# google-research/multinerf

Measured on NVIDIA H100. Metric: train-step rays/sec @16384 rays x (64+64+32) samples, higher is better.
Workload: dtype bf16

## Files before the change

### include/mnrf.h

```cpp
#ifndef MNRF_H_
#define MNRF_H_

#include <stddef.h>
#include <stdint.h>

#ifdef __cplusplus
extern "C" {
#endif

typedef uint16_t mnrf_bf16;
typedef void* mnrf_stream;

#define MNRF_ABI_VERSION 2

int mnrf_abi_version(void);
const char* mnrf_last_error(void);
int mnrf_device_ok(void);
int mnrf_num_sms(void);

typedef struct {
  int32_t num_rays, num_prev, num_samples;
  int32_t use_dilation;
  float dilation, domain_lo, domain_hi;
  float anneal, resample_padding;
// ... 54 lines not shown
                    const float* side_w, float* side_aw, float* out, mnrf_stream stream);

typedef struct {
  int32_t block_n;
  int32_t staged;
  int32_t mask_tma;
  int32_t smooth;
  int32_t side;
  int32_t splits;
  int32_t tiles;
  int32_t grid;
  int32_t pingpong;
  int32_t epilogue;
} mnrf_gemm_instance;
int mnrf_gemm_plan(const mnrf_gemm_desc* d, const mnrf_bf16* a, const mnrf_bf16* b, const float* bias,
                   const float* rowv, const float* colv, const mnrf_bf16* mask, const uint32_t* maskbits,
                   const float* colsum, const mnrf_bf16* addend, const mnrf_bf16* z, int64_t ldz, const void* out,
                   const float* bsum, const float* side_w, const float* side_aw, mnrf_gemm_instance* plan);

#define MNRF_CHAIN_MAX_LAYERS 8
enum { MNRF_CHAIN_FWD = 0, MNRF_CHAIN_BWD = 1 };

typedef struct {
  const mnrf_bf16* w;
  int64_t ldw;
  const float* bias;
  uint32_t* maskbits;
  int64_t ldmaskbits;
  float* colsum;
  mnrf_bf16* out;
  int64_t ldo;
  int32_t n_stream, stream_col0, stream_kb0;
  int32_t n_res, res_kb0;
  int32_t reserved;
} mnrf_chain_layer;

typedef struct {
  int32_t mode, num_layers;
  int32_t width;
  int32_t stream_cols;
  int64_t m;
  const mnrf_bf16* stream;
  int64_t ldstream;
  const float* head_w;
  const float* head_b;
  float* head_out;
  int32_t head_n;
  int32_t reserved;
  mnrf_chain_layer layer[MNRF_CHAIN_MAX_LAYERS];
} mnrf_chain_desc;

int mnrf_mlp_chain(const mnrf_chain_desc* d, mnrf_stream stream);
int mnrf_mlp_chain_max_layers(void);

int mnrf_head_fwd(int64_t m, int32_t k, int32_t n_out, const mnrf_bf16* x, int64_t ldx,
                  const mnrf_bf16* w, const float* b, float* raw, mnrf_stream stream);
int mnrf_head_bwd(int64_t m, int32_t k, int32_t n_out, const mnrf_bf16* x, int64_t ldx,
                  const mnrf_bf16* w, const float* draw, mnrf_bf16* dx, int64_t lddx,
                  int32_t act, const mnrf_bf16* z, int64_t ldz, float* dw, float* dw2, int32_t dw_split,
                  float* db, float* dxsum, int32_t dx_cols, mnrf_bf16* dx2, int64_t lddx2, mnrf_stream stream);

enum { MNRF_HEAD_NONE = 0, MNRF_HEAD_FWD_SUB = 1, MNRF_HEAD_FWD_WARP = 2, MNRF_HEAD_BWD_SUB = 3,
       MNRF_HEAD_BWD_WARP = 4 };
typedef struct {
  int32_t fwd_kernel;
  int32_t fwd_lpr;
  int32_t fwd_grid;
  int32_t bwd_kernel;
  int32_t bwd_n_out;
  int32_t bwd_lpr;
  int32_t bwd_chunks;
  int32_t bwd_smooth;
  int32_t bwd_grid;
  int32_t reserved;
  int64_t fwd_rows_per_pass;
  int64_t bwd_rows_per_block;
} mnrf_head_instance;
int mnrf_head_plan(int64_t m, int32_t k, int32_t n_out, const mnrf_bf16* x, const mnrf_bf16* w, int32_t act,
                   const mnrf_bf16* z, const mnrf_bf16* dx, mnrf_head_instance* plan);

int mnrf_colsum(int64_t m, int32_t n, const mnrf_bf16* x, int64_t ldx, float* out,
                mnrf_stream stream);

enum { MNRF_RGB_SIGMOID = 0, MNRF_RGB_SAFE_EXP = 1 };

typedef struct {
  int32_t num_rays, num_samples;
  int32_t raydist_fn, opaque_background;
  float density_bias, density_noise;
  int32_t rgb_act;
  float rgb_premult, rgb_bias, rgb_padding;
  float bg_const;
  int32_t rgb_mode;
  int32_t ld_density, ld_rgb;
} mnrf_composite_desc;

int mnrf_composite_fwd(const mnrf_composite_desc* d, const float* raw_density,
                       const float* raw_rgb, const float* density_noise, const float* sdist,
                       const float* directions, const float* near, const float* far,
                       const float* bg_rgb, const float* rgb_scale, const float* raw_diffuse,
                       const float* raw_tint, float* weights, float* rgb_out,
                       float* density_out, float* rgb_samples, float* acc, float* dist,
                       mnrf_stream stream);

int mnrf_point_rgb(const mnrf_composite_desc* d, int64_t M, const float* raw_rgb, int32_t ld_rgb,
                   const float* raw_diffuse, const float* raw_tint, float* rgb_out, mnrf_stream stream);
// ... 198 lines not shown
```

### multinerf_b200/csrc/chain.cu

```cuda
#include <stdlib.h>
#include <string.h>

#include <algorithm>

#include "tc_common.cuh"

namespace mnrf {

constexpr int CH_W = 256;
constexpr int CH_ROWS = 128;
constexpr int CH_KBLK = CH_ROWS * 128;
constexpr int CH_WBLK = CH_W * 128;
constexpr int CH_RING = 4;
constexpr int CH_SEG = CH_W / 64;
constexpr int CH_SBLK = 64 * 128;
constexpr int CH_SRING = 3;
constexpr int CH_ACT = 4 * CH_KBLK;
constexpr int CH_THREADS = 384;
constexpr int CH_MAX_LAYERS = MNRF_CHAIN_MAX_LAYERS;
constexpr int CH_AUX = CH_MAX_LAYERS * CH_W * 4;
constexpr int CH_SMEM = CH_ACT + CH_RING * CH_WBLK + CH_SRING * CH_SBLK + CH_AUX + 256  + 1024 ;
static_assert(CH_SMEM <= 232448, "shared memory budget");
static_assert(CH_SEG >= 1 && CH_SEG <= CH_RING, "a segment must fit in the weight ring");

struct alignas(64) ChainMaps {
  CUtensorMap stream;
  CUtensorMap w[CH_MAX_LAYERS];
  CUtensorMap out[CH_MAX_LAYERS];
};

struct ChainLayer {
  int n_stream, stream_col0, stream_kb0;
  int n_res, res_kb0;
  int store;
  const float* bias;
  uint32_t* maskbits;
  int64_t ldmaskbits;
  float* colsum;
};

struct ChainParams {
  int num_layers;
  int64_t m;
  int64_t num_units;
  ChainLayer layer[CH_MAX_LAYERS];
  const float* head_w;
  const float* head_b;
  float* head_out;
};

__device__ __forceinline__ uint32_t pack_bf16_relu(float lo, float hi) {
  uint32_t r;
  asm("cvt.rn.relu.bf16x2.f32 %0, %1, %2;" : "=r"(r) : "f"(hi), "f"(lo));
  return r;
}

__device__ __forceinline__ float2 ld_shared_const_f2(uint32_t addr) {
  float2 v;
  asm("ld.shared.v2.f32 {%0, %1}, [%2];" : "=f"(v.x), "=f"(v.y) : "r"(addr));
  return v;
}

enum { CK_TURN, CK_FULL, CK_MMA, CK_EPI_SYNC, CK_EPI_LOOP, CK_EPI_TAIL, CK_N };
#ifdef MNRF_CHAIN_CLOCKS
__device__ unsigned long long g_chain_clk[CK_N];
#define CH_CLK(k) do { const long long t_ = clock64(); clk[k] += t_ - clk_t; clk_t = t_; } while (0)
#else
#define CH_CLK(k) do { } while (0)
#endif

template <int MODE, int NH>
__global__ void __launch_bounds__(CH_THREADS, 1)
mlp_chain_kernel(const __grid_constant__ ChainMaps maps, const ChainParams p) {
  extern __shared__ uint8_t smem_dyn[];
  uint8_t* smem = reinterpret_cast<uint8_t*>((reinterpret_cast<uintptr_t>(smem_dyn) + 1023) & ~uintptr_t(1023));
  uint8_t* act = smem;
  uint8_t* wring = act + CH_ACT;
  uint8_t* sring = wring + CH_RING * CH_WBLK;
  float* aux = reinterpret_cast<float*>(sring + CH_SRING * CH_SBLK);
  uint64_t* wfull = reinterpret_cast<uint64_t*>(aux + CH_MAX_LAYERS * CH_W);
  uint64_t* wempty = wfull + CH_RING;
  uint64_t* sfull = wempty + CH_RING;
  uint64_t* sempty = sfull + CH_SRING;
  uint64_t* turn = sempty + CH_SRING;

  const int warp = threadIdx.x >> 5;
  const int lane = threadIdx.x & 31;
  const int wg = threadIdx.x >> 7;

  if (threadIdx.x == 0) {
    bool any_stream = false;
    for (int j = 0; j < p.num_layers; ++j) {
      prefetch_tmap(&maps.w[j]);
      if (p.layer[j].store) prefetch_tmap(&maps.out[j]);
      any_stream |= p.layer[j].n_stream > 0;
    }
    if (any_stream) prefetch_tmap(&maps.stream);
    for (int i = 0; i < CH_RING; ++i) { mbar_init(&wfull[i], 1); mbar_init(&wempty[i], 8); }
    for (int i = 0; i < CH_SRING; ++i) { mbar_init(&sfull[i], 1); mbar_init(&sempty[i], 4); }
    for (int i = 0; i < 2; ++i) mbar_init(&turn[i], 4);
    fence_barrier_init();
  }
  if (MODE == 1)
    for (int i = threadIdx.x; i < CH_MAX_LAYERS * CH_W; i += CH_THREADS) aux[i] = 0.f;
  __syncthreads();
  pdl_launch_dependents();
  pdl_wait();
  if (MODE == 0) {
    for (int i = threadIdx.x; i < p.num_layers * CH_W; i += CH_THREADS) aux[i] = __ldg(p.layer[i / CH_W].bias + i % CH_W);
    __syncthreads();
  }

  if (wg == 0) {
    setmaxnreg_dec<40>();
    if (threadIdx.x == 0) {
      uint32_t wslot = 0, wphase = 0, sslot = 0, sphase = 0;
      for (int64_t unit = blockIdx.x; unit < p.num_units; unit += gridDim.x) {
        const int row0 = (int)(unit * CH_ROWS);
        for (int j = 0; j < p.num_layers; ++j) {
          const ChainLayer& L = p.layer[j];
          const int nk = L.n_res + L.n_stream;
          for (int s0 = 0; s0 < nk; s0 += CH_SEG) {
            const int s1 = min(s0 + CH_SEG, nk);
            for (int c = 0; c < 2; ++c)
              for (int s = s0; s < s1; ++s) {
                const bool streamed = s >= L.n_res;
                const int si = s - L.n_res;
                if (c == 0) {
                  mbar_wait(&wempty[wslot], wphase ^ 1, 1);
                  mbar_expect_tx(&wfull[wslot], CH_WBLK);
                  tma_load_2d(wring + wslot * CH_WBLK, &maps.w[j], &wfull[wslot],
                              (streamed ? L.stream_kb0 + si : L.res_kb0 + s) * 64, 0);
                  if (++wslot == CH_RING) { wslot = 0; wphase ^= 1; }
                }
                if (streamed) {
                  mbar_wait(&sempty[sslot], sphase ^ 1, 2);
                  mbar_expect_tx(&sfull[sslot], CH_SBLK);
                  tma_load_2d(sring + sslot * CH_SBLK, &maps.stream, &sfull[sslot], L.stream_col0 + si * 64, row0 + 64 * c);
                  if (++sslot == CH_SRING) { sslot = 0; sphase ^= 1; }
                }
              }
          }
          if (j == 0 && L.n_stream > 0 && unit + gridDim.x < p.num_units)
            for (int si = 0; si < L.n_stream; ++si)
              for (int c = 0; c < 2; ++c)
                tma_prefetch_2d(&maps.stream, L.stream_col0 + si * 64, (int)((unit + gridDim.x) * CH_ROWS) + 64 * c);
        }
      }
    }
  } else {
    setmaxnreg_inc<232>();
    const int c = wg - 1;
    const int w = warp & 3;
    const int r_in = 64 * c + 16 * w + (lane >> 2);
    const int q = lane & 3;
    const int cq = 2 * q;
    const uint32_t wring_s = smem_u32(wring), sring_s = smem_u32(sring), act_s = smem_u32(act);
    const uint32_t aux_s = smem_u32(aux);
    const bool lead = (threadIdx.x & 127) == 0;
    uint32_t wslot = 0, wphase = 0;
    uint32_t spos = 0;
    uint32_t seg = 0;
#ifdef MNRF_CHAIN_CLOCKS
    long long clk[CK_N] = {};
    long long clk_t = clock64();
#endif
    float acc[CH_W / 2];
    for (int64_t unit = blockIdx.x; unit < p.num_units; unit += gridDim.x) {
      int64_t rows[2];
      bool row_ok[2];
#pragma unroll
      for (int h = 0; h < 2; ++h) {
        rows[h] = unit * CH_ROWS + r_in + 8 * h;
        row_ok[h] = rows[h] < p.m;
      }
      for (int j = 0; j < p.num_layers; ++j) {
        const ChainLayer& L = p.layer[j];
        const bool last = (j == p.num_layers - 1);
        const bool do_head = (MODE == 0) && last && p.head_w != nullptr;
        uint32_t mw[2][2] = {{0u, 0u}, {0u, 0u}};
        if (MODE == 1 && L.maskbits) {
#pragma unroll
          for (int h = 0; h < 2; ++h)
#pragma unroll
            for (int e = 0; e < 2; ++e)
              if (row_ok[h]) mw[h][e] = __ldg(L.maskbits + rows[h] * L.ldmaskbits + 2 * q + e);
        }
        const int nk = L.n_res + L.n_stream;
        fence_acc(acc);
        for (int s0 = 0; s0 < nk; s0 += CH_SEG, ++seg) {
          const int s1 = min(s0 + CH_SEG, nk);
          const int ns = s1 - max(s0, L.n_res);
          uint32_t sp = spos + (c && ns > 0 ? ns : 0);
          if (ns > 0) spos += 2 * ns;
          if (c == 1) mbar_wait(&turn[1], seg & 1, 7);
          else if (seg > 0) mbar_wait(&turn[0], (seg - 1) & 1, 7);
          CH_CLK(CK_TURN);
          int prev_w = -1, prev_s = -1;
          for (int s = s0; s < s1; ++s) {
            const bool streamed = s >= L.n_res;
            mbar_wait(&wfull[wslot], wphase, 3);
            uint32_t a0 = act_s + s * CH_KBLK + c * (64 * 128);
            int cur_s = -1;
            if (streamed) {
              cur_s = (int)(sp % CH_SRING);
              mbar_wait(&sfull[cur_s], (sp / CH_SRING) & 1, 4);
              a0 = sring_s + cur_s * CH_SBLK;
              ++sp;
            }
            CH_CLK(CK_FULL);
            const uint32_t b0 = wring_s + wslot * CH_WBLK;
            wgmma_fence();
#pragma unroll
            for (int k = 0; k < 64 / WGMMA_K; ++k)
              Wgmma<CH_W, 0, 0>::mma(acc, make_smem_desc(a0 + k * (WGMMA_K * 2), 0, 1024),
                                     make_smem_desc(b0 + k * (WGMMA_K * 2), 0, 1024), (s > 0 || k > 0) ? 1u : 0u);
            wgmma_commit();
            wgmma_wait<1>();
            if (lane == 0) {
              if (prev_w >= 0) mbar_arrive(&wempty[prev_w]);
              if (prev_s >= 0) mbar_arrive(&sempty[prev_s]);
            }
            prev_w = (int)wslot;
            prev_s = cur_s;
            if (++wslot == CH_RING) { wslot = 0; wphase ^= 1; }
          }
          __syncwarp();
          if (lane == 0) mbar_arrive(&turn[c ^ 1]);
          wgmma_wait<0>();
          if (lane == 0) {
            mbar_arrive(&wempty[prev_w]);
            if (prev_s >= 0) mbar_arrive(&sempty[prev_s]);
          }
          CH_CLK(CK_MMA);
        }
        fence_acc(acc);

        if (lead) tma_store_wait_read<0>();
        named_bar_sync(1 + c, 128);
        CH_CLK(CK_EPI_SYNC);
        uint32_t bits[2] = {0u, 0u};
        float hdot[NH][2];
#pragma unroll
        for (int o = 0; o < NH; ++o) hdot[o][0] = hdot[o][1] = 0.f;
#pragma unroll
        for (int i = 0; i < CH_W / 8; ++i) {
          const int col = 8 * i + cq;
          float v[2][2];
#pragma unroll
          for (int h = 0; h < 2; ++h) { v[h][0] = acc[4 * i + 2 * h]; v[h][1] = acc[4 * i + 2 * h + 1]; }
          uint32_t o[2];
          if (MODE == 0) {
            const float2 b = ld_shared_const_f2(aux_s + (j * CH_W + col) * 4);
#pragma unroll
            for (int h = 0; h < 2; ++h) {
              v[h][0] += b.x;
              v[h][1] += b.y;
              bits[h] |= ((v[h][0] > 0.f ? 1u : 0u) | (v[h][1] > 0.f ? 2u : 0u)) << (col & 31);
              o[h] = pack_bf16_relu(v[h][0], v[h][1]);
            }
            if (do_head) {
#pragma unroll
              for (int oo = 0; oo < NH; ++oo) {
                const float2 hw = __ldg(reinterpret_cast<const float2*>(p.head_w + oo * CH_W + col));
#pragma unroll
                for (int h = 0; h < 2; ++h) hdot[oo][h] += bf16_lo(o[h]) * hw.x + bf16_hi(o[h]) * hw.y;
              }
            }
          } else {
            if (L.maskbits && (i & 3) == 0) {
#pragma unroll
              for (int h = 0; h < 2; ++h)
                bits[h] = __shfl_sync(0xffffffffu, mw[h][(i >> 2) & 1], (lane & ~3) | (i >> 3));
            }
#pragma unroll
            for (int h = 0; h < 2; ++h) {
              if (L.maskbits) {
                if (!((bits[h] >> (col & 31)) & 1u)) v[h][0] = 0.f;
                if (!((bits[h] >> ((col + 1) & 31)) & 1u)) v[h][1] = 0.f;
              }
              o[h] = pack_bf16(v[h][0], v[h][1]);
            }
            if (L.colsum) {
              float s0 = v[0][0] + v[1][0], s1 = v[0][1] + v[1][1];
#pragma unroll
              for (int sh = 4; sh < 32; sh <<= 1) {
                s0 += __shfl_xor_sync(0xffffffffu, s0, sh);
                s1 += __shfl_xor_sync(0xffffffffu, s1, sh);
              }
              if (lane < 4) { atomicAdd(aux + j * CH_W + col, s0); atomicAdd(aux + j * CH_W + col + 1, s1); }
            }
          }
#pragma unroll
          for (int h = 0; h < 2; ++h) {
            const int r = r_in + 8 * h;
            st_shared_u32(act_s + (col >> 6) * CH_KBLK + r * 128 + ((((col & 63) >> 3) ^ (r & 7)) << 4) + (cq << 1), o[h]);
          }
          if (MODE == 0 && (i & 3) == 3) {
#pragma unroll
            for (int h = 0; h < 2; ++h) {
              bits[h] |= __shfl_xor_sync(0xffffffffu, bits[h], 1);
              bits[h] |= __shfl_xor_sync(0xffffffffu, bits[h], 2);
              if (q == (i >> 3)) mw[h][(i >> 2) & 1] = bits[h];
              bits[h] = 0u;
            }
          }
        }
        CH_CLK(CK_EPI_LOOP);
        fence_proxy_async();
        named_bar_sync(1 + c, 128);
        CH_CLK(CK_EPI_SYNC);
        if (lead && L.store) {
#pragma unroll
          for (int kb = 0; kb < 4; ++kb)
            tma_store_2d(&maps.out[j], act + kb * CH_KBLK + c * (64 * 128), kb * 64, (int)(unit * CH_ROWS) + 64 * c);
          tma_store_commit();
        }
        if (MODE == 0 && L.maskbits) {
          const bool wide = (((uintptr_t)L.maskbits | (uintptr_t)(L.ldmaskbits * 4)) & 7) == 0;
#pragma unroll
          for (int h = 0; h < 2; ++h) {
            if (!row_ok[h]) continue;
            uint32_t* dst = L.maskbits + rows[h] * L.ldmaskbits + 2 * q;
            if (wide) *reinterpret_cast<uint2*>(dst) = make_uint2(mw[h][0], mw[h][1]);
            else { dst[0] = mw[h][0]; dst[1] = mw[h][1]; }
          }
        }
        if (do_head) {
#pragma unroll
          for (int oo = 0; oo < NH; ++oo)
#pragma unroll
            for (int h = 0; h < 2; ++h) {
              hdot[oo][h] += __shfl_xor_sync(0xffffffffu, hdot[oo][h], 1);
              hdot[oo][h] += __shfl_xor_sync(0xffffffffu, hdot[oo][h], 2);
              if (q == 0 && row_ok[h])
                p.head_out[rows[h] * NH + oo] = hdot[oo][h] + (p.head_b ? __ldg(p.head_b + oo) : 0.f);
            }
        }
        CH_CLK(CK_EPI_TAIL);
      }
    }
    if (lead) tma_store_wait_all();
#ifdef MNRF_CHAIN_CLOCKS
    if (blockIdx.x == 0 && threadIdx.x == 256)
      for (int k = 0; k < CK_N; ++k) atomicAdd(&g_chain_clk[k], (unsigned long long)clk[k]);
#endif
    if (MODE == 1) {
      named_bar_sync(3, 256);
      for (int jj = 0; jj < p.num_layers; ++jj) {
        if (!p.layer[jj].colsum) continue;
        for (int i = threadIdx.x - 128; i < CH_W; i += 256) atomicAdd(p.layer[jj].colsum + i, aux[jj * CH_W + i]);
      }
    }
  }
}

}

extern "C" int mnrf_mlp_chain_max_layers(void) { return mnrf::CH_MAX_LAYERS; }

#ifdef MNRF_CHAIN_CLOCKS
extern "C" int mnrf_chain_clocks(unsigned long long* out) {
  unsigned long long zero[mnrf::CK_N] = {};
  if (cudaDeviceSynchronize() != cudaSuccess) return 1;
  if (cudaMemcpyFromSymbol(out, mnrf::g_chain_clk, sizeof(zero)) != cudaSuccess) return 1;
  return cudaMemcpyToSymbol(mnrf::g_chain_clk, zero, sizeof(zero)) != cudaSuccess;
}
#endif

extern "C" int mnrf_mlp_chain(const mnrf_chain_desc* d, mnrf_stream stream_) {
  using namespace mnrf;
  cudaStream_t stream = (cudaStream_t)stream_;
  MNRF_CHECK(d, "mnrf_mlp_chain: null descriptor");
  MNRF_CHECK(d->m >= 0 && (d->m + CH_ROWS - 1) / CH_ROWS * CH_ROWS <= INT32_MAX,
             "mnrf_mlp_chain: m must be in [0, %d], got %lld", INT32_MAX / CH_ROWS * CH_ROWS, (long long)d->m);
  if (d->m == 0) return 0;
  MNRF_CHECK(d->mode == MNRF_CHAIN_FWD || d->mode == MNRF_CHAIN_BWD, "mnrf_mlp_chain: bad mode %d", d->mode);
  MNRF_CHECK(d->num_layers >= 1 && d->num_layers <= CH_MAX_LAYERS, "mnrf_mlp_chain: 1..%d layers, got %d",
             CH_MAX_LAYERS, d->num_layers);
  MNRF_CHECK(d->width == CH_W, "mnrf_mlp_chain: layer width must be %d, got %d", CH_W, d->width);
  const int sms = mnrf_num_sms();
  ChainMaps maps;
  memset(&maps, 0, sizeof(maps));
  ChainParams p{};
  p.num_layers = d->num_layers;
  p.m = d->m;
  p.num_units = (d->m + CH_ROWS - 1) / CH_ROWS;
  bool any_stream = false;
  for (int j = 0; j < d->num_layers; ++j) {
    const mnrf_chain_layer& s = d->layer[j];
    ChainLayer& L = p.layer[j];
    MNRF_CHECK(s.n_res == 0 || s.n_res == CH_W / 64, "mnrf_mlp_chain: layer %d: n_res must be 0 or %d", j, CH_W / 64);
    MNRF_CHECK(s.n_stream >= 0 && (s.n_stream > 0 || s.n_res > 0), "mnrf_mlp_chain: layer %d has no operand", j);
    MNRF_CHECK(s.stream_col0 >= 0 && s.stream_kb0 >= 0 && s.res_kb0 >= 0,
               "mnrf_mlp_chain: layer %d: negative column or k-block offset", j);
    MNRF_CHECK(j > 0 || s.n_res == 0, "mnrf_mlp_chain: the first layer has no resident operand");
    MNRF_CHECK(s.w && ((uintptr_t)s.w % 16) == 0 && s.ldw % 8 == 0, "mnrf_mlp_chain: layer %d: weights must be 16-byte aligned", j);
    const int kblocks = std::max(s.n_stream > 0 ? s.stream_kb0 + s.n_stream : 0, s.n_res > 0 ? s.res_kb0 + s.n_res : 0);
    MNRF_CHECK(s.ldw >= (int64_t)kblocks * 64, "mnrf_mlp_chain: layer %d: weight pitch %lld < K %d", j, (long long)s.ldw, kblocks * 64);
    L.n_stream = s.n_stream; L.stream_col0 = s.stream_col0; L.stream_kb0 = s.stream_kb0;
    L.n_res = s.n_res; L.res_kb0 = s.res_kb0;
    L.store = s.out ? 1 : 0;
    L.bias = s.bias; L.maskbits = s.maskbits; L.ldmaskbits = s.ldmaskbits; L.colsum = s.colsum;
    if (s.bias) MNRF_CHECK(((uintptr_t)s.bias % 8) == 0, "mnrf_mlp_chain: layer %d: bias must be 8-byte aligned", j);
    if (s.maskbits)
      MNRF_CHECK(s.ldmaskbits >= CH_W / 32, "mnrf_mlp_chain: layer %d: maskbits rows must hold >= %d words", j, CH_W / 32);
    if (d->mode == MNRF_CHAIN_BWD) MNRF_CHECK(!s.bias, "mnrf_mlp_chain: bias is a forward input");
    else MNRF_CHECK(s.bias && !s.colsum, "mnrf_mlp_chain: layer %d: the forward chain takes a bias and no colsum", j);
    if (make_tmap(&maps.w[j], s.w, CH_W, (int64_t)kblocks * 64, s.ldw, 64, CH_W)) return 1;
    if (s.out) {
      MNRF_CHECK(((uintptr_t)s.out % 16) == 0 && s.ldo % 8 == 0 && s.ldo >= CH_W, "mnrf_mlp_chain: layer %d: output alignment", j);
      if (make_tmap(&maps.out[j], s.out, d->m, CH_W, s.ldo, 64, 64)) return 1;
    }
    any_stream |= s.n_stream > 0;
    if (s.n_stream > 0)
      MNRF_CHECK(s.stream_col0 % 64 == 0 && s.stream_col0 + s.n_stream * 64 <= d->stream_cols,
                 "mnrf_mlp_chain: layer %d: streamed columns [%d, %d) outside the stream tensor (%d columns)", j,
                 s.stream_col0, s.stream_col0 + s.n_stream * 64, d->stream_cols);
  }
  if (any_stream) {
    MNRF_CHECK(d->stream && ((uintptr_t)d->stream % 16) == 0 && d->ldstream % 8 == 0 && d->stream_cols % 64 == 0,
               "mnrf_mlp_chain: streamed operand must be 16-byte aligned with a multiple of 64 columns");
    MNRF_CHECK(d->ldstream >= d->stream_cols, "mnrf_mlp_chain: stream pitch %lld < %d columns",
               (long long)d->ldstream, d->stream_cols);
    if (make_tmap(&maps.stream, d->stream, d->m, d->stream_cols, d->ldstream, 64, CH_ROWS / 2)) return 1;
  }
  p.head_w = d->head_w; p.head_b = d->head_b; p.head_out = d->head_out;
  const int head_n = d->head_n ? d->head_n : 1;
  if (d->head_w) MNRF_CHECK(d->mode == MNRF_CHAIN_FWD && d->head_out && ((uintptr_t)d->head_w % 16) == 0,
                            "mnrf_mlp_chain: the head is a forward output (16-byte aligned weights)");
  MNRF_CHECK(head_n == 1 || (head_n == 4 && d->head_w), "mnrf_mlp_chain: head_n must be 1 or 4, got %d", head_n);
  const int grid = (int)std::min<int64_t>(p.num_units, sms);
  const int rc = d->mode == MNRF_CHAIN_BWD ? launch_tc<mlp_chain_kernel<1, 1>>(grid, CH_THREADS, CH_SMEM, stream, maps, p)
                 : head_n == 4             ? launch_tc<mlp_chain_kernel<0, 4>>(grid, CH_THREADS, CH_SMEM, stream, maps, p)
                                           : launch_tc<mlp_chain_kernel<0, 1>>(grid, CH_THREADS, CH_SMEM, stream, maps, p);
  if (rc) return rc;
  MNRF_LAUNCH_CHECK();
  return 0;
}
```

### multinerf_b200/lib.py

```python
import ctypes as C
import os

import torch

_HERE = os.path.dirname(os.path.abspath(__file__))
LIB_PATH = os.environ.get('MNRF_LIB') or os.path.join(_HERE, 'libmnrf_b200.so')


class MnrfError(RuntimeError):
  pass


class SampleDesc(C.Structure):
  _fields_ = [('num_rays', C.c_int32), ('num_prev', C.c_int32), ('num_samples', C.c_int32),
              ('use_dilation', C.c_int32), ('dilation', C.c_float), ('domain_lo', C.c_float),
              ('domain_hi', C.c_float), ('anneal', C.c_float), ('resample_padding', C.c_float),
              ('jitter_mode', C.c_int32), ('max_jitter', C.c_float)]


class EncodeDesc(C.Structure):
  _fields_ = [('num_rays', C.c_int32), ('num_samples', C.c_int32), ('raydist_fn', C.c_int32),
              ('ray_shape', C.c_int32), ('warp_contract', C.c_int32),
              ('disable_integration', C.c_int32), ('basis_k', C.c_int32), ('min_deg', C.c_int32),
              ('max_deg', C.c_int32), ('ld_feat', C.c_int32), ('feat_cols', C.c_int32)]
# ... 32 lines not shown
  _fields_ = [('c', CompositeDesc), ('loss_type', C.c_int32), ('charb_padding', C.c_float),
              ('data_mult', C.c_float), ('distortion_mult', C.c_float),
              ('interlevel_mult', C.c_float), ('num_samples_fine', C.c_int32),
              ('lossmult_channels', C.c_int32)]


class RobustDesc(C.Structure):
  _fields_ = [('num_rays', C.c_int32), ('patch_size', C.c_int32), ('inner_patch_size', C.c_int32),
              ('filter_size', C.c_int32), ('enable', C.c_int32), ('smoothed_thresh', C.c_float),
              ('patch_thresh', C.c_float)]


class RefdirDesc(C.Structure):
  _fields_ = [('M', C.c_int64), ('num_samples', C.c_int32), ('use_pred_normals', C.c_int32),
              ('use_density_normals', C.c_int32), ('use_reflections', C.c_int32), ('use_ide', C.c_int32),
              ('use_n_dot_v', C.c_int32), ('use_roughness', C.c_int32), ('deg_view', C.c_int32),
              ('ide_n', C.c_int32), ('roughness_bias', C.c_float), ('ld', C.c_int32), ('col0', C.c_int32),
              ('col_end', C.c_int32)]


class CameraDesc(C.Structure):
  _fields_ = [('num_rays', C.c_int32), ('num_cameras', C.c_int32), ('camtype', C.c_int32),
              ('has_distortion', C.c_int32), ('k1', C.c_float), ('k2', C.c_float), ('k3', C.c_float),
              ('k4', C.c_float), ('p1', C.c_float), ('p2', C.c_float), ('undistort_eps', C.c_float),
              ('undistort_iters', C.c_int32), ('has_ndc', C.c_int32), ('ndc_p02', C.c_float),
              ('ndc_p12', C.c_float), ('ndc_near', C.c_float)]


class SphericalDesc(C.Structure):
  _fields_ = [('height', C.c_int32), ('width', C.c_int32), ('camtoworld', C.c_double * 12)]


class PackItem(C.Structure):
  _fields_ = [('master', C.c_void_p), ('w_nk', C.c_void_p), ('w_kn', C.c_void_p), ('in_pad', C.c_int32),
              ('out', C.c_int32), ('tile0', C.c_int32), ('reserved', C.c_int32)]


CHAIN_MAX_LAYERS = 8
CHAIN_FWD, CHAIN_BWD = 0, 1


class ChainLayer(C.Structure):
  _fields_ = [('w', C.c_void_p), ('ldw', C.c_int64), ('bias', C.c_void_p), ('maskbits', C.c_void_p),
              ('ldmaskbits', C.c_int64), ('colsum', C.c_void_p), ('out', C.c_void_p), ('ldo', C.c_int64),
              ('n_stream', C.c_int32), ('stream_col0', C.c_int32), ('stream_kb0', C.c_int32),
              ('n_res', C.c_int32), ('res_kb0', C.c_int32), ('reserved', C.c_int32)]


class ChainDesc(C.Structure):
  _fields_ = [('mode', C.c_int32), ('num_layers', C.c_int32), ('width', C.c_int32), ('stream_cols', C.c_int32),
              ('m', C.c_int64), ('stream', C.c_void_p), ('ldstream', C.c_int64), ('head_w', C.c_void_p),
              ('head_b', C.c_void_p), ('head_out', C.c_void_p), ('head_n', C.c_int32), ('reserved', C.c_int32),
              ('layer', ChainLayer * CHAIN_MAX_LAYERS)]


class AdamDesc(C.Structure):
  _fields_ = [('n', C.c_int64), ('grad_max_val', C.c_float), ('grad_max_norm', C.c_float),
              ('lr', C.c_float), ('beta1', C.c_float), ('beta2', C.c_float), ('eps', C.c_float),
              ('step', C.c_int32), ('grad_scale', C.c_float)]


RAYDIST = {None: 0, 'none': 0, 'reciprocal': 1, 'log': 2, 'exp': 3, 'sqrt': 4, 'square': 5,
           'piecewise': 6}
RAY_SHAPE = {'cone': 0, 'cylinder': 1}
RGB_ACT = {'sigmoid': 0, 'safe_exp': 1}
LOSS_TYPE = {'mse': 0, 'charb': 1, 'rawnerf': 2}
GEMM_FWD, GEMM_DGRAD, GEMM_WGRAD = 0, 1, 2
ACT_NONE, ACT_RELU, ACT_SOFTPLUS, ACT_SILU = 0, 1, 2, 3
SMOOTH_ACTS = (ACT_SOFTPLUS, ACT_SILU)

_P = C.c_void_p
_SIGNATURES = {
    'mnrf_abi_version': (C.c_int, []),
    'mnrf_last_error': (C.c_char_p, []),
    'mnrf_device_ok': (C.c_int, []),
    'mnrf_num_sms': (C.c_int, []),
    'mnrf_sample_level': (C.c_int, [C.POINTER(SampleDesc)] + [_P] * 12),
    'mnrf_encode': (C.c_int, [C.POINTER(EncodeDesc)] + [_P] * 11 + [C.c_int32, _P]),
    'mnrf_viewdir_enc': (C.c_int, [C.c_int32, C.c_int32, C.c_int32, _P, _P, C.c_int32, C.c_int32,
                                   C.c_int32, _P]),
    'mnrf_gemm': (C.c_int, [C.POINTER(GemmDesc)] + [_P] * 10 + [C.c_int64, _P, _P]),
    'mnrf_gemm_wgrad': (C.c_int, [C.POINTER(GemmDesc)] + [_P] * 7),
    'mnrf_gemm_plan': (C.c_int, [C.POINTER(GemmDesc)] + [_P] * 10 + [C.c_int64] + [_P] * 4 +
                       [C.POINTER(GemmInstance)]),
    'mnrf_mlp_chain': (C.c_int, [C.POINTER(ChainDesc), _P]),
    'mnrf_mlp_chain_max_layers': (C.c_int, []),
    'mnrf_head_fwd': (C.c_int, [C.c_int64, C.c_int32, C.c_int32, _P, C.c_int64, _P, _P, _P, _P]),
    'mnrf_head_bwd': (C.c_int, [C.c_int64, C.c_int32, C.c_int32, _P, C.c_int64, _P, _P, _P, C.c_int64, C.c_int32,
                                _P, C.c_int64, _P, _P, C.c_int32, _P, _P, C.c_int32, _P, C.c_int64, _P]),
    'mnrf_head_plan': (C.c_int, [C.c_int64, C.c_int32, C.c_int32, _P, _P, C.c_int32, _P, _P, _P]),
    'mnrf_colsum': (C.c_int, [C.c_int64, C.c_int32, _P, C.c_int64, _P, _P]),
    'mnrf_composite_fwd': (C.c_int, [C.POINTER(CompositeDesc)] + [_P] * 18),
    'mnrf_composite_bwd': (C.c_int, [C.POINTER(LossDesc)] + [_P] * 24 + [C.c_int32, _P]),
    'mnrf_robust_mask': (C.c_int, [C.POINTER(RobustDesc)] + [_P] * 7 + [C.c_int32, _P]),
    'mnrf_quantile': (C.c_int, [C.c_int32, C.c_float, _P, _P, _P]),
    'mnrf_refdir_fwd': (C.c_int, [C.POINTER(RefdirDesc)] + [_P] * 10 + [C.c_float, C.c_float, C.c_int32, _P, _P]),
    'mnrf_refdir_bwd': (C.c_int, [C.POINTER(RefdirDesc)] + [_P] * 8 + [C.c_int32, C.c_float, C.c_float, C.c_int32] +
                        [_P] * 8),
    'mnrf_normals_fwd': (C.c_int, [C.c_int64, C.c_int32] + [_P] * 5 + [C.c_float, C.c_float, C.c_int32, _P, _P]),
    'mnrf_normals_bwd': (C.c_int, [C.c_int64, C.c_int32] + [_P] * 4 + [C.c_float, C.c_float, C.c_int32] + [_P] * 2 +
                         [C.c_int64] + [_P] * 3 +
                         [C.c_int64, _P, _P]),
    'mnrf_outer_mask': (C.c_int,[C.c_int64, C.c_int32, C.c_int64, _P, _P, _P, C.c_int64, _P, C.c_int64, _P]),
    'mnrf_act_tangent_bwd': (C.c_int, [C.c_int64, C.c_int32, C.c_int32] + [_P, C.c_int64] * 5 + [C.c_int32, _P]),
    'mnrf_pixels_to_rays': (C.c_int, [C.POINTER(CameraDesc)] + [_P] * 11),
    'mnrf_spherical_rays': (C.c_int, [C.POINTER(SphericalDesc)] + [_P] * 6),
    'mnrf_clip_adam': (C.c_int, [C.POINTER(AdamDesc)] + [_P] * 7),
    'mnrf_pack_weights_batched': (C.c_int, [C.c_int32, _P, C.c_int32, _P]),
    'mnrf_encode_points': (C.c_int, [C.POINTER(EncodeDesc), _P, C.c_float, _P, _P, _P, _P]),
    'mnrf_marching_cubes': (C.c_int, [C.c_int32] * 4 + [_P, C.c_float] + [_P] * 7),
    'mnrf_encode_points_tangent': (C.c_int, [C.POINTER(EncodeDesc), _P, C.c_float, _P, _P, _P, C.c_int32, _P]),
    'mnrf_point_rgb': (C.c_int, [C.POINTER(CompositeDesc), C.c_int64, _P, C.c_int32, _P, _P, _P, _P]),
    'mnrf_mc_normals': (C.c_int, [C.c_int32] * 3 + [_P, C.c_float] + [_P] * 4),
    'mnrf_tsdf_integrate': (C.c_int, [C.POINTER(CameraDesc)] + [C.c_int32] * 3 + [C.c_double] * 4 + [C.c_int32] * 3 +
                            [_P] * 5 + [C.c_float] + [_P] * 5),
    'mnrf_tsdf_integrate_contracted': (C.c_int, [C.POINTER(CameraDesc)] + [C.c_int32] * 3 + [C.c_double] * 4 +
                                       [C.c_int32] * 3 + [_P] * 5 + [C.c_float] + [_P] * 5),
    'mnrf_mesh_uncontract': (C.c_int, [C.c_int64] + [_P] * 5),
    'mnrf_mesh_components': (C.c_int, [C.c_int32, C.c_int64, _P, _P, _P]),
    'mnrf_points_view_count': (C.c_int, [C.POINTER(CameraDesc), C.c_int64, _P, C.c_int32, C.c_int32, C.c_int32,
                                         _P, _P, _P, _P]),
    'mnrf_mesh_quadrics': (C.c_int, [C.c_int32, C.c_int64] + [_P] * 4 + [C.c_int64] + [_P] * 6),
    'mnrf_mesh_edge_cost': (C.c_int, [C.c_int32, C.c_int64, C.c_int64] + [_P] * 12),
    'mnrf_mesh_collapse_select': (C.c_int, [C.c_int32, C.c_int64, C.c_int64] + [_P] * 7),
    'mnrf_mesh_collapse_apply': (C.c_int, [C.c_int32, C.c_int64, C.c_int64] + [_P] * 13),
    'mnrf_mesh_texture_raster': (C.c_int, [C.c_int32, C.c_int64, _P, _P, _P, C.c_int32] + [_P] * 5),
    'mnrf_mesh_bvh': (C.c_int, [C.c_int32, C.c_int32, C.c_int64] + [_P] * 12),
    'mnrf_mesh_trace': (C.c_int, [C.c_int64] + [_P] * 4 + [C.c_int64] + [_P] * 9),
}
MC_COUNT, MC_EMIT = 0, 1
BVH_BOXES, BVH_KEYS, BVH_TREE = 0, 1, 2
HEAD_NONE, HEAD_FWD_SUB, HEAD_FWD_WARP, HEAD_BWD_SUB, HEAD_BWD_WARP = 0, 1, 2, 3, 4
EXPORTED = tuple(_SIGNATURES)

_lib = None


def load(build_if_missing=False):
  global _lib
# ... 45 lines not shown
```

### multinerf_b200/ops.py

```python
import ctypes as C
import math
from typing import NamedTuple

import torch

from . import lib as L

EPS = float(torch.finfo(torch.float32).eps)

LAUNCHES = 0
GEMM_EVENTS = None


def _count(n=1):
  global LAUNCHES
  LAUNCHES += n


def _gemm_call(flops, fn, *args):
  _count()
  if GEMM_EVENTS is None:
    L.check(fn(*args))
    return
  ev = (torch.cuda.Event(enable_timing=True), torch.cuda.Event(enable_timing=True))
# ... 433 lines not shown
  _gemm_call(2.0 * m * n * k, lib.mnrf_gemm_wgrad, C.byref(d), L.ptr(x), L.ptr(dy), L.ptr(bsum),
             L.ptr(_f32(side_w)), L.ptr(side_aw), L.ptr(out), L.stream_ptr())
  return out


def gemm_plan(mode, a, b, out, *, m, n, k, act=L.ACT_NONE, bias=None, rowv=None, colv=None, mask=None,
              maskbits=None, colsum=None, mask_mod=0, addend=None, z=None, bsum=None, side_w=None, side_aw=None):
  lib = L.load()
  def p(t):
    return None if t is None else C.c_void_p(t.data_ptr())
  def ld(t):
    return t.stride(0) if t is not None else 0
  d = L.GemmDesc(mode, act, m, n, k, a.stride(0), b.stride(0), out.stride(0), ld(mask), ld(maskbits), ld(addend),
                 mask_mod, 0)
  plan = L.GemmInstance()
  L.check(lib.mnrf_gemm_plan(C.byref(d), p(a), p(b), p(bias), p(rowv), p(colv), p(mask), p(maskbits), p(colsum),
                             p(addend), p(z), ld(z), p(out), p(bsum), p(side_w), p(side_aw), C.byref(plan)))
  return {name: int(getattr(plan, name)) for name, _ in L.GemmInstance._fields_}


def chain_desc(mode, m, layers, *, stream=None, stream_cols=0, head_w=None, head_b=None, head_out=None, head_n=1):
  d = L.ChainDesc()
  d.mode, d.num_layers, d.width, d.stream_cols, d.m = mode, len(layers), 256, stream_cols, m
  if stream is not None:
    assert stream.dtype == torch.bfloat16 and stream.stride(1) == 1
    d.stream, d.ldstream = stream.data_ptr(), stream.stride(0)
  if head_w is not None:
    assert head_w.is_contiguous() and head_w.numel() == head_n * 256 and head_out.is_contiguous()
    d.head_w, d.head_out, d.head_n = head_w.data_ptr(), head_out.data_ptr(), head_n
    d.head_b = head_b.data_ptr() if head_b is not None else None
  flops = 0.0
  for j, ly in enumerate(layers):
    c = d.layer[j]
    w = ly['w']
    assert w.dtype == torch.bfloat16 and w.stride(1) == 1
    c.w, c.ldw = w.data_ptr(), w.stride(0)
    for name in ('bias', 'colsum'):
      t = ly.get(name)
      setattr(c, name, t.data_ptr() if t is not None else None)
    mb = ly.get('maskbits')
    if mb is not None:
      assert mb.dtype == torch.int32 and mb.stride(1) == 1
      c.maskbits, c.ldmaskbits = mb.data_ptr(), mb.stride(0)
    out = ly.get('out')
    if out is not None:
      assert out.dtype == torch.bfloat16 and out.stride(1) == 1
      c.out, c.ldo = out.data_ptr(), out.stride(0)
    c.n_stream, c.stream_col0, c.stream_kb0 = ly.get('n_stream', 0), ly.get('stream_col0', 0), ly.get('stream_kb0', 0)
    c.n_res, c.res_kb0 = ly.get('n_res', 0), ly.get('res_kb0', 0)
    flops += 2.0 * m * 256 * 64 * (c.n_stream + c.n_res)
  return d, flops


def mlp_chain(desc):
  lib = L.load()
  d, flops = desc
  _gemm_call(flops, lib.mnrf_mlp_chain, C.byref(d), L.stream_ptr())


def head_fwd(x, w_nk, bias, n_out, k, raw=None):
  lib = L.load()
  M = x.shape[0]
  if raw is None:
    raw = torch.empty(M, n_out, device=x.device)
  _count()
  L.check(lib.mnrf_head_fwd(M, k, n_out, L.ptr(x), x.stride(0), L.ptr(w_nk), L.ptr(bias),
                            L.ptr(raw), L.stream_ptr()))
  return raw


def head_bwd(x, w_nk, draw, n_out, k, dx=None, relu_mask=False, dw=None, db=None, dxsum=None, dw2=None, dw_split=0,
             dx_cols=0, dx2=None, act=L.ACT_NONE, z=None):
  lib = L.load()
  M = x.shape[0]
  if z is not None:
    assert not relu_mask and z.dtype == torch.bfloat16 and z.stride(-1) == 1
  else:
    act = L.ACT_RELU if relu_mask else L.ACT_NONE
  _count()
  L.check(lib.mnrf_head_bwd(M, k, n_out, L.ptr(x), x.stride(0), L.ptr(w_nk), L.ptr(_f32(draw)),
                            L.ptr(dx), dx.stride(0) if dx is not None else 0, act,
                            L.ptr(z), z.stride(0) if z is not None else 0, L.ptr(dw), L.ptr(dw2), int(dw_split),
                            L.ptr(db), L.ptr(dxsum), int(dx_cols), L.ptr(dx2), dx2.stride(0) if dx2 is not None else 0,
                            L.stream_ptr()))


def head_plan(x, w_nk, n_out, k, *, act=L.ACT_NONE, z=None, dx=None):
  lib = L.load()
  def p(t):
    return None if t is None else C.c_void_p(t.data_ptr())
  plan = L.HeadInstance()
  L.check(lib.mnrf_head_plan(x.shape[0], k, n_out, p(x), p(w_nk), act, p(z), p(dx), C.byref(plan)))
  return {name: int(getattr(plan, name)) for name, _ in L.HeadInstance._fields_}


def colsum(x, n, out):
  lib = L.load()
  _count()
  L.check(lib.mnrf_colsum(x.shape[0], n, L.ptr(x), x.stride(0), L.ptr(out), L.stream_ptr()))


def _cdesc(B, S, *, raydist_fn, opaque_background, density_bias, density_noise, rgb_activation,
           rgb_premultiplier, rgb_bias, rgb_padding, bg_const, rgb_mode=0):
  if rgb_activation not in L.RGB_ACT:
    raise ValueError(f'rgb_activation {rgb_activation!r} not supported by the CUDA path')
  return L.CompositeDesc(B, S, L.RAYDIST[raydist_fn], int(opaque_background), float(density_bias),
# ... 214 lines not shown
```

Measured before the change: 293,300.

## Specialize backward chain epilogue for mask-only layers with TMA-loaded mask bits

Adds a template variant of the fused MLP chain kernel for backward passes where every layer has relu mask bits and no column sums. Mask words are prefetched per layer by the producer warp via TMA into a double-buffered shared area guarded by mbarriers, replacing per-thread global loads and shuffles. The column-sum zeroing and reduction are also compiled out. This adds barrier traffic and reuses the aux area, and falls back to an LDG variant when alignment does not allow TMA.

```diff
diff --git a/include/mnrf.h b/include/mnrf.h
--- a/include/mnrf.h
+++ b/include/mnrf.h
@@ -130,6 +130,12 @@
 
 int mnrf_mlp_chain(const mnrf_chain_desc* d, mnrf_stream stream);
 int mnrf_mlp_chain_max_layers(void);
+
+enum { MNRF_CHAIN_EPI_GENERIC = 0, MNRF_CHAIN_EPI_BITS = 1 };
+typedef struct {
+  int32_t epilogue, mask_tma, head_n, reserved;
+} mnrf_chain_instance;
+int mnrf_chain_plan(const mnrf_chain_desc* d, mnrf_chain_instance* plan);
 
 int mnrf_head_fwd(int64_t m, int32_t k, int32_t n_out, const mnrf_bf16* x, int64_t ldx,
                   const mnrf_bf16* w, const float* b, float* raw, mnrf_stream stream);
diff --git a/multinerf_b200/csrc/chain.cu b/multinerf_b200/csrc/chain.cu
--- a/multinerf_b200/csrc/chain.cu
+++ b/multinerf_b200/csrc/chain.cu
@@ -19,14 +19,22 @@
 constexpr int CH_THREADS = 384;
 constexpr int CH_MAX_LAYERS = MNRF_CHAIN_MAX_LAYERS;
 constexpr int CH_AUX = CH_MAX_LAYERS * CH_W * 4;
+constexpr int CH_MWORDS = CH_W / 32;
+constexpr int CH_MBLK = CH_ROWS * CH_MWORDS * 4;
+constexpr int CH_MBUFS = 2;
+static_assert(CH_MBUFS * CH_MBLK <= CH_AUX, "the mask blocks live in the column-sum area");
 constexpr int CH_SMEM = CH_ACT + CH_RING * CH_WBLK + CH_SRING * CH_SBLK + CH_AUX + 256  + 1024 ;
 static_assert(CH_SMEM <= 232448, "shared memory budget");
+static_assert((2 * CH_RING + 2 * CH_SRING + 2 + 2 * CH_MBUFS) * 8 <= 256, "barrier area");
+
+enum { CH_EPI_GENERIC = 0, CH_EPI_BITS_TMA = 1, CH_EPI_BITS_LDG = 2 };
 static_assert(CH_SEG >= 1 && CH_SEG <= CH_RING, "a segment must fit in the weight ring");
 
 struct alignas(64) ChainMaps {
   CUtensorMap stream;
   CUtensorMap w[CH_MAX_LAYERS];
   CUtensorMap out[CH_MAX_LAYERS];
+  CUtensorMap mask[CH_MAX_LAYERS];
 };
 
 struct ChainLayer {
@@ -69,9 +77,12 @@
 #define CH_CLK(k) do { } while (0)
 #endif
 
-template <int MODE, int NH>
+template <int MODE, int NH, int OPS>
 __global__ void __launch_bounds__(CH_THREADS, 1)
 mlp_chain_kernel(const __grid_constant__ ChainMaps maps, const ChainParams p) {
+  static_assert(OPS == CH_EPI_GENERIC || (MODE == 1 && NH == 1), "fixed operand sets are backward epilogues");
+  constexpr bool kFixed = OPS != CH_EPI_GENERIC;
+  constexpr bool kBitsTma = OPS == CH_EPI_BITS_TMA;
   extern __shared__ uint8_t smem_dyn[];
   uint8_t* smem = reinterpret_cast<uint8_t*>((reinterpret_cast<uintptr_t>(smem_dyn) + 1023) & ~uintptr_t(1023));
   uint8_t* act = smem;
@@ -83,6 +94,8 @@
   uint64_t* sfull = wempty + CH_RING;
   uint64_t* sempty = sfull + CH_SRING;
   uint64_t* turn = sempty + CH_SRING;
+  uint64_t* mfull = turn + 2;
+  uint64_t* mempty = mfull + CH_MBUFS;
 
   const int warp = threadIdx.x >> 5;
   const int lane = threadIdx.x & 31;
@@ -93,15 +106,18 @@
     for (int j = 0; j < p.num_layers; ++j) {
       prefetch_tmap(&maps.w[j]);
       if (p.layer[j].store) prefetch_tmap(&maps.out[j]);
+      if (kBitsTma) prefetch_tmap(&maps.mask[j]);
       any_stream |= p.layer[j].n_stream > 0;
     }
     if (any_stream) prefetch_tmap(&maps.stream);
     for (int i = 0; i < CH_RING; ++i) { mbar_init(&wfull[i], 1); mbar_init(&wempty[i], 8); }
     for (int i = 0; i < CH_SRING; ++i) { mbar_init(&sfull[i], 1); mbar_init(&sempty[i], 4); }
     for (int i = 0; i < 2; ++i) mbar_init(&turn[i], 4);
+    if (kBitsTma)
+      for (int i = 0; i < CH_MBUFS; ++i) { mbar_init(&mfull[i], 1); mbar_init(&mempty[i], 8); }
     fence_barrier_init();
   }
-  if (MODE == 1)
+  if (MODE == 1 && !kFixed)
     for (int i = threadIdx.x; i < CH_MAX_LAYERS * CH_W; i += CH_THREADS) aux[i] = 0.f;
   __syncthreads();
   pdl_launch_dependents();
@@ -115,11 +131,18 @@
     setmaxnreg_dec<40>();
     if (threadIdx.x == 0) {
       uint32_t wslot = 0, wphase = 0, sslot = 0, sphase = 0;
+      uint32_t g = 0;
       for (int64_t unit = blockIdx.x; unit < p.num_units; unit += gridDim.x) {
         const int row0 = (int)(unit * CH_ROWS);
-        for (int j = 0; j < p.num_layers; ++j) {
+        for (int j = 0; j < p.num_layers; ++j, ++g) {
           const ChainLayer& L = p.layer[j];
           const int nk = L.n_res + L.n_stream;
+          if (kBitsTma) {
+            const uint32_t mb = g % CH_MBUFS;
+            mbar_wait(&mempty[mb], ((g / CH_MBUFS) & 1) ^ 1, 5);
+            mbar_expect_tx(&mfull[mb], CH_MBLK);
+            tma_load_2d(reinterpret_cast<uint8_t*>(aux) + mb * CH_MBLK, &maps.mask[j], &mfull[mb], 0, row0);
+          }
           for (int s0 = 0; s0 < nk; s0 += CH_SEG) {
             const int s1 = min(s0 + CH_SEG, nk);
             for (int c = 0; c < 2; ++c)
@@ -161,6 +184,7 @@
     uint32_t wslot = 0, wphase = 0;
     uint32_t spos = 0;
     uint32_t seg = 0;
+    uint32_t g = 0;
 #ifdef MNRF_CHAIN_CLOCKS
     long long clk[CK_N] = {};
     long long clk_t = clock64();
@@ -174,12 +198,14 @@
         rows[h] = unit * CH_ROWS + r_in + 8 * h;
         row_ok[h] = rows[h] < p.m;
       }
-      for (int j = 0; j < p.num_layers; ++j) {
+      for (int j = 0; j < p.num_layers; ++j, ++g) {
         const ChainLayer& L = p.layer[j];
         const bool last = (j == p.num_layers - 1);
         const bool do_head = (MODE == 0) && last && p.head_w != nullptr;
+        const bool has_bits = kFixed || L.maskbits != nullptr;
+        const bool has_colsum = !kFixed && L.colsum != nullptr;
         uint32_t mw[2][2] = {{0u, 0u}, {0u, 0u}};
-        if (MODE == 1 && L.maskbits) {
+        if (MODE == 1 && !kBitsTma && has_bits) {
 #pragma unroll
           for (int h = 0; h < 2; ++h)
 #pragma unroll
@@ -237,6 +263,8 @@
         fence_acc(acc);
 
         if (lead) tma_store_wait_read<0>();
+        const uint32_t m_row = aux_s + (g % CH_MBUFS) * CH_MBLK + r_in * (CH_MWORDS * 4);
+        if (kBitsTma) mbar_wait(&mfull[g % CH_MBUFS], (g / CH_MBUFS) & 1, 6);
         named_bar_sync(1 + c, 128);
         CH_CLK(CK_EPI_SYNC);
         uint32_t bits[2] = {0u, 0u};
@@ -268,20 +296,26 @@
               }
             }
           } else {
-            if (L.maskbits && (i & 3) == 0) {
-#pragma unroll
-              for (int h = 0; h < 2; ++h)
-                bits[h] = __shfl_sync(0xffffffffu, mw[h][(i >> 2) & 1], (lane & ~3) | (i >> 3));
+            if (has_bits && (i & 3) == 0) {
+#pragma unroll
+              for (int h = 0; h < 2; ++h) {
+                bits[h] = kBitsTma ? ld_shared_u32(m_row + (8 * h * CH_MWORDS + (i >> 2)) * 4)
+                                   : __shfl_sync(0xffffffffu, mw[h][(i >> 2) & 1], (lane & ~3) | (i >> 3));
+                if (kFixed) bits[h] >>= cq;
+              }
             }
 #pragma unroll
             for (int h = 0; h < 2; ++h) {
-              if (L.maskbits) {
+              if (kFixed) {
+                if (!(bits[h] & (1u << (8 * (i & 3))))) v[h][0] = 0.f;
+                if (!(bits[h] & (2u << (8 * (i & 3))))) v[h][1] = 0.f;
+              } else if (has_bits) {
                 if (!((bits[h] >> (col & 31)) & 1u)) v[h][0] = 0.f;
                 if (!((bits[h] >> ((col + 1) & 31)) & 1u)) v[h][1] = 0.f;
               }
               o[h] = pack_bf16(v[h][0], v[h][1]);
             }
-            if (L.colsum) {
+            if (has_colsum) {
               float s0 = v[0][0] + v[1][0], s1 = v[0][1] + v[1][1];
 #pragma unroll
               for (int sh = 4; sh < 32; sh <<= 1) {
@@ -305,6 +339,10 @@
               bits[h] = 0u;
             }
           }
+        }
+        if (kBitsTma) {
+          __syncwarp();
+          if (lane == 0) mbar_arrive(&mempty[g % CH_MBUFS]);
         }
         CH_CLK(CK_EPI_LOOP);
         fence_proxy_async();
@@ -345,7 +383,7 @@
     if (blockIdx.x == 0 && threadIdx.x == 256)
       for (int k = 0; k < CK_N; ++k) atomicAdd(&g_chain_clk[k], (unsigned long long)clk[k]);
 #endif
-    if (MODE == 1) {
+    if (MODE == 1 && !kFixed) {
       named_bar_sync(3, 256);
       for (int jj = 0; jj < p.num_layers; ++jj) {
         if (!p.layer[jj].colsum) continue;
@@ -368,25 +406,20 @@
 }
 #endif
 
-extern "C" int mnrf_mlp_chain(const mnrf_chain_desc* d, mnrf_stream stream_) {
-  using namespace mnrf;
-  cudaStream_t stream = (cudaStream_t)stream_;
-  MNRF_CHECK(d, "mnrf_mlp_chain: null descriptor");
-  MNRF_CHECK(d->m >= 0 && (d->m + CH_ROWS - 1) / CH_ROWS * CH_ROWS <= INT32_MAX,
-             "mnrf_mlp_chain: m must be in [0, %d], got %lld", INT32_MAX / CH_ROWS * CH_ROWS, (long long)d->m);
-  if (d->m == 0) return 0;
+namespace mnrf {
+
+static int chain_setup(const mnrf_chain_desc* d, ChainParams* pp, mnrf_chain_instance* plan) {
   MNRF_CHECK(d->mode == MNRF_CHAIN_FWD || d->mode == MNRF_CHAIN_BWD, "mnrf_mlp_chain: bad mode %d", d->mode);
   MNRF_CHECK(d->num_layers >= 1 && d->num_layers <= CH_MAX_LAYERS, "mnrf_mlp_chain: 1..%d layers, got %d",
              CH_MAX_LAYERS, d->num_layers);
   MNRF_CHECK(d->width == CH_W, "mnrf_mlp_chain: layer width must be %d, got %d", CH_W, d->width);
-  const int sms = mnrf_num_sms();
-  ChainMaps maps;
-  memset(&maps, 0, sizeof(maps));
-  ChainParams p{};
+  ChainParams& p = *pp;
+  p = ChainParams{};
   p.num_layers = d->num_layers;
   p.m = d->m;
   p.num_units = (d->m + CH_ROWS - 1) / CH_ROWS;
   bool any_stream = false;
+  bool bits_only = d->mode == MNRF_CHAIN_BWD, bits_tma = bits_only;
   for (int j = 0; j < d->num_layers; ++j) {
     const mnrf_chain_layer& s = d->layer[j];
     ChainLayer& L = p.layer[j];
@@ -407,33 +440,79 @@
       MNRF_CHECK(s.ldmaskbits >= CH_W / 32, "mnrf_mlp_chain: layer %d: maskbits rows must hold >= %d words", j, CH_W / 32);
     if (d->mode == MNRF_CHAIN_BWD) MNRF_CHECK(!s.bias, "mnrf_mlp_chain: bias is a forward input");
     else MNRF_CHECK(s.bias && !s.colsum, "mnrf_mlp_chain: layer %d: the forward chain takes a bias and no colsum", j);
-    if (make_tmap(&maps.w[j], s.w, CH_W, (int64_t)kblocks * 64, s.ldw, 64, CH_W)) return 1;
-    if (s.out) {
+    if (s.out)
       MNRF_CHECK(((uintptr_t)s.out % 16) == 0 && s.ldo % 8 == 0 && s.ldo >= CH_W, "mnrf_mlp_chain: layer %d: output alignment", j);
-      if (make_tmap(&maps.out[j], s.out, d->m, CH_W, s.ldo, 64, 64)) return 1;
-    }
     any_stream |= s.n_stream > 0;
     if (s.n_stream > 0)
       MNRF_CHECK(s.stream_col0 % 64 == 0 && s.stream_col0 + s.n_stream * 64 <= d->stream_cols,
                  "mnrf_mlp_chain: layer %d: streamed columns [%d, %d) outside the stream tensor (%d columns)", j,
                  s.stream_col0, s.stream_col0 + s.n_stream * 64, d->stream_cols);
+    bits_only = bits_only && s.maskbits && !s.colsum;
+    bits_tma = bits_tma && ((uintptr_t)s.maskbits % 16) == 0 && s.ldmaskbits % 4 == 0;
   }
   if (any_stream) {
     MNRF_CHECK(d->stream && ((uintptr_t)d->stream % 16) == 0 && d->ldstream % 8 == 0 && d->stream_cols % 64 == 0,
                "mnrf_mlp_chain: streamed operand must be 16-byte aligned with a multiple of 64 columns");
     MNRF_CHECK(d->ldstream >= d->stream_cols, "mnrf_mlp_chain: stream pitch %lld < %d columns",
                (long long)d->ldstream, d->stream_cols);
-    if (make_tmap(&maps.stream, d->stream, d->m, d->stream_cols, d->ldstream, 64, CH_ROWS / 2)) return 1;
   }
   p.head_w = d->head_w; p.head_b = d->head_b; p.head_out = d->head_out;
   const int head_n = d->head_n ? d->head_n : 1;
   if (d->head_w) MNRF_CHECK(d->mode == MNRF_CHAIN_FWD && d->head_out && ((uintptr_t)d->head_w % 16) == 0,
                             "mnrf_mlp_chain: the head is a forward output (16-byte aligned weights)");
   MNRF_CHECK(head_n == 1 || (head_n == 4 && d->head_w), "mnrf_mlp_chain: head_n must be 1 or 4, got %d", head_n);
-  const int grid = (int)std::min<int64_t>(p.num_units, sms);
-  const int rc = d->mode == MNRF_CHAIN_BWD ? launch_tc<mlp_chain_kernel<1, 1>>(grid, CH_THREADS, CH_SMEM, stream, maps, p)
-                 : head_n == 4             ? launch_tc<mlp_chain_kernel<0, 4>>(grid, CH_THREADS, CH_SMEM, stream, maps, p)
-                                           : launch_tc<mlp_chain_kernel<0, 1>>(grid, CH_THREADS, CH_SMEM, stream, maps, p);
+  plan->epilogue = bits_only ? MNRF_CHAIN_EPI_BITS : MNRF_CHAIN_EPI_GENERIC;
+  plan->mask_tma = bits_only && bits_tma;
+  plan->head_n = d->mode == MNRF_CHAIN_FWD ? head_n : 0;
+  plan->reserved = 0;
+  return 0;
+}
+
+}
+
+extern "C" int mnrf_chain_plan(const mnrf_chain_desc* d, mnrf_chain_instance* plan) {
+  MNRF_CHECK(d && plan, "mnrf_chain_plan: null pointer");
+  MNRF_CHECK(d->m > 0 && (d->m + mnrf::CH_ROWS - 1) / mnrf::CH_ROWS * mnrf::CH_ROWS <= INT32_MAX,
+             "mnrf_chain_plan: m must be in [1, %d] (an empty launch runs no kernel), got %lld",
+             INT32_MAX / mnrf::CH_ROWS * mnrf::CH_ROWS, (long long)d->m);
+  mnrf::ChainParams p;
+  return mnrf::chain_setup(d, &p, plan);
+}
+
+extern "C" int mnrf_mlp_chain(const mnrf_chain_desc* d, mnrf_stream stream_) {
+  using namespace mnrf;
+  cudaStream_t stream = (cudaStream_t)stream_;
+  MNRF_CHECK(d, "mnrf_mlp_chain: null descriptor");
+  MNRF_CHECK(d->m >= 0 && (d->m + CH_ROWS - 1) / CH_ROWS * CH_ROWS <= INT32_MAX,
+             "mnrf_mlp_chain: m must be in [0, %d], got %lld", INT32_MAX / CH_ROWS * CH_ROWS, (long long)d->m);
+  if (d->m == 0) return 0;
+  ChainParams p;
+  mnrf_chain_instance plan;
+  if (int rc = chain_setup(d, &p, &plan)) return rc;
+  ChainMaps maps;
+  memset(&maps, 0, sizeof(maps));
+  for (int j = 0; j < d->num_layers; ++j) {
+    const mnrf_chain_layer& s = d->layer[j];
+    const int kblocks = std::max(s.n_stream > 0 ? s.stream_kb0 + s.n_stream : 0, s.n_res > 0 ? s.res_kb0 + s.n_res : 0);
+    if (make_tmap(&maps.w[j], s.w, CH_W, (int64_t)kblocks * 64, s.ldw, 64, CH_W)) return 1;
+    if (s.out && make_tmap(&maps.out[j], s.out, d->m, CH_W, s.ldo, 64, 64)) return 1;
+    if (plan.mask_tma && make_tmap(&maps.mask[j], s.maskbits, d->m, CH_MWORDS, s.ldmaskbits, CH_MWORDS, CH_ROWS,
+                                   CU_TENSOR_MAP_DATA_TYPE_UINT32, 4, CU_TENSOR_MAP_SWIZZLE_NONE))
+      return 1;
+  }
+  if (std::any_of(p.layer, p.layer + p.num_layers, [](const ChainLayer& L) { return L.n_stream > 0; }) &&
+      make_tmap(&maps.stream, d->stream, d->m, d->stream_cols, d->ldstream, 64, CH_ROWS / 2))
+    return 1;
+  const int grid = (int)std::min<int64_t>(p.num_units, mnrf_num_sms());
+  int rc;
+  if (d->mode == MNRF_CHAIN_BWD)
+    rc = plan.epilogue == MNRF_CHAIN_EPI_GENERIC
+             ? launch_tc<mlp_chain_kernel<1, 1, CH_EPI_GENERIC>>(grid, CH_THREADS, CH_SMEM, stream, maps, p)
+         : plan.mask_tma ? launch_tc<mlp_chain_kernel<1, 1, CH_EPI_BITS_TMA>>(grid, CH_THREADS, CH_SMEM, stream, maps, p)
+                         : launch_tc<mlp_chain_kernel<1, 1, CH_EPI_BITS_LDG>>(grid, CH_THREADS, CH_SMEM, stream, maps, p);
+  else
+    rc = plan.head_n == 4 ? launch_tc<mlp_chain_kernel<0, 4, CH_EPI_GENERIC>>(grid, CH_THREADS, CH_SMEM, stream, maps, p)
+                          : launch_tc<mlp_chain_kernel<0, 1, CH_EPI_GENERIC>>(grid, CH_THREADS, CH_SMEM, stream, maps, p);
   if (rc) return rc;
   MNRF_LAUNCH_CHECK();
   return 0;
diff --git a/multinerf_b200/lib.py b/multinerf_b200/lib.py
--- a/multinerf_b200/lib.py
+++ b/multinerf_b200/lib.py
@@ -108,6 +108,13 @@
               ('m', C.c_int64), ('stream', C.c_void_p), ('ldstream', C.c_int64), ('head_w', C.c_void_p),
               ('head_b', C.c_void_p), ('head_out', C.c_void_p), ('head_n', C.c_int32), ('reserved', C.c_int32),
               ('layer', ChainLayer * CHAIN_MAX_LAYERS)]
+
+
+class ChainInstance(C.Structure):
+  _fields_ = [('epilogue', C.c_int32), ('mask_tma', C.c_int32), ('head_n', C.c_int32), ('reserved', C.c_int32)]
+
+
+CHAIN_EPI_GENERIC, CHAIN_EPI_BITS = 0, 1
 
 
 class AdamDesc(C.Structure):
@@ -141,6 +148,7 @@
                        [C.POINTER(GemmInstance)]),
     'mnrf_mlp_chain': (C.c_int, [C.POINTER(ChainDesc), _P]),
     'mnrf_mlp_chain_max_layers': (C.c_int, []),
+    'mnrf_chain_plan': (C.c_int, [C.POINTER(ChainDesc), _P]),
     'mnrf_head_fwd': (C.c_int, [C.c_int64, C.c_int32, C.c_int32, _P, C.c_int64, _P, _P, _P, _P]),
     'mnrf_head_bwd': (C.c_int, [C.c_int64, C.c_int32, C.c_int32, _P, C.c_int64, _P, _P, _P, C.c_int64, C.c_int32,
                                 _P, C.c_int64, _P, _P, C.c_int32, _P, _P, C.c_int32, _P, C.c_int64, _P]),
diff --git a/multinerf_b200/ops.py b/multinerf_b200/ops.py
--- a/multinerf_b200/ops.py
+++ b/multinerf_b200/ops.py
@@ -509,6 +509,13 @@
   return d, flops
 
 
+def chain_plan(desc):
+  lib = L.load()
+  plan = L.ChainInstance()
+  L.check(lib.mnrf_chain_plan(C.byref(desc[0]), C.byref(plan)))
+  return {name: int(getattr(plan, name)) for name, _ in L.ChainInstance._fields_}
+
+
 def mlp_chain(desc):
   lib = L.load()
   d, flops = desc
```

After: 297,200, median of 6. 1.3% higher.
